# Aceinna/gnss-ins-sim

Hardware: NVIDIA H100
Metric: MC-runs x timesteps/sec free_integration @100Hz (higher is better)
Workload: dtype f64

## Files before the change

gnss_ins_sim_b200/csrc/b2ins_api.cu:

```cuda
#include <cmath>
#include <cstdarg>
#include <cstdio>
#include <cstdlib>
#include <cstring>
#include <limits>
#include <vector>

#include "../../include/b2ins.h"
#include "allan_kernel.cuh"
#include "internal.h"
#include "noise_kernel.cuh"
#include "pathgen_host.h"
#include "psd_kernel.cuh"
#include "gps_kernel.cuh"
#include "mag_kernel.cuh"
#include "ekf_kernel.cuh"
#include "stats_kernel.cuh"
#include "sensor_stats_kernel.cuh"

#ifdef B2INS_SINGLE_TU
#define B2_RF 0
#define B2_PLAIN_NAME launch_mc_plain_rf0
#define B2_SPEC_NAME launch_mc_spec_rf0
#include "mc_plain_launch.cuh"
// ... 860 lines not shown
    p.p0[3 + c] = cfg->gps_stdv[c] * cfg->gps_stdv[c];
    p.p0[6 + c] = cfg->ini_att_std[c] * cfg->ini_att_std[c];
    p.p0[9 + c] = cfg->gyro_err.b_drift[c] * cfg->gyro_err.b_drift[c] + cfg->gyro_err.b[c] * cfg->gyro_err.b[c];
    p.p0[12 + c] = cfg->accel_err.b_drift[c] * cfg->accel_err.b_drift[c] + cfg->accel_err.b[c] * cfg->accel_err.b[c];
    const bool wg = std::isinf(cfg->gyro_err.b_corr[c]), wa = std::isinf(cfg->accel_err.b_corr[c]);
    p.ag[c] = wg ? 0.0 : p.gyro.gm_a[c];
    p.qg[c] = wg ? p.gyro.wd[c] * p.gyro.wd[c] : p.gyro.gm_b[c] * p.gyro.gm_b[c];
    p.aa[c] = wa ? 0.0 : p.accel.gm_a[c];
    p.qa[c] = wa ? p.accel.wd[c] * p.accel.wd[c] : p.accel.gm_b[c] * p.accel.gm_b[c];
    p.arw2dt[c] = cfg->gyro_err.rw[c] * cfg->gyro_err.rw[c] * p.dt;
    p.vrw2dt[c] = cfg->accel_err.rw[c] * cfg->accel_err.rw[c] * p.dt;
  }
  for (int c = 0; c < 9; ++c) p.ini[c] = cfg->ini[c];
  ARG_CHECK(cfg->vel_rw >= 0.0 && cfg->att_rw >= 0.0, "vel_rw and att_rw must be >= 0");
  p.qv_extra = cfg->vel_rw * cfg->vel_rw * p.dt;
  p.qphi_extra = cfg->att_rw * cfg->att_rw * p.dt;
  p.stats_start = cfg->stats_start;
  p.end_err = end_err;
  p.end_bias = end_bias;
  p.consist = consist;
  p.out_att = dump_att;
  p.out_pos = dump_pos;
  p.out_vel = dump_vel;
  p.out_wb = dump_wb;
  p.out_ab = dump_ab;
  p.dump_runs = ndump ? cfg->dump_runs : 0;
  p.dump_stride = cfg->dump_stride > 1 ? cfg->dump_stride : 1;
  p.dump_rows = (cfg->n + p.dump_stride - 1) / p.dump_stride;
  const unsigned grid = static_cast<unsigned>((cfg->runs + kEkfRuns - 1) / kEkfRuns);
  ekf_kernel<<<grid, kEkfThreads, 0, static_cast<cudaStream_t>(stream)>>>(p);
  CU_CHECK(cudaGetLastError());
  return B2INS_OK;
}

int64_t b2ins_error_stats_workspace_bytes(int ncomp) {
  if (ncomp < 1) return 0;
  return static_cast<int64_t>(sizeof(double)) * (static_cast<int64_t>(kStatBlocks) * 2 + 4) * ncomp;
}

static int stage1_grid(int64_t runs, int ncomp, int threads) {
  const int64_t total = runs * ncomp;
  int64_t g = (total + threads - 1) / threads;
  if (g > kStatBlocks) g = kStatBlocks;
  if (g < 1) g = 1;
  return static_cast<int>(g);
}

int b2ins_error_partial_f64(int64_t runs, int ncomp, const double* err, double* partial,
                            void* workspace, void* stream) {
  ARG_CHECK(runs > 0 && ncomp >= 1 && ncomp <= kStatMaxComp, "bad runs/ncomp");
  ARG_CHECK(err && partial && workspace, "null buffer");
  cudaStream_t s = static_cast<cudaStream_t>(stream);
  const int threads = stat_threads(ncomp);
  const int grid = stage1_grid(runs, ncomp, threads);
  double* ws = static_cast<double*>(workspace);
  err_stage1_kernel<0><<<grid, threads, 2 * threads * sizeof(double), s>>>(runs, ncomp, err,
                                                                           nullptr, ws);
  err_stage2_kernel<0><<<1, 32, 0, s>>>(grid, ncomp, ws, partial);
  CU_CHECK(cudaGetLastError());
  return B2INS_OK;
}

int b2ins_error_partial2_f64(int64_t runs, int ncomp, const double* err, const double* mean,
                             double* partial2, void* workspace, void* stream) {
  ARG_CHECK(runs > 0 && ncomp >= 1 && ncomp <= kStatMaxComp, "bad runs/ncomp");
  ARG_CHECK(err && mean && partial2 && workspace, "null buffer");
  cudaStream_t s = static_cast<cudaStream_t>(stream);
  const int threads = stat_threads(ncomp);
  const int grid = stage1_grid(runs, ncomp, threads);
  double* ws = static_cast<double*>(workspace);
  err_stage1_kernel<1><<<grid, threads, 2 * threads * sizeof(double), s>>>(runs, ncomp, err, mean,
                                                                           ws);
  err_stage2_kernel<1><<<1, 32, 0, s>>>(grid, ncomp, ws, partial2);
  CU_CHECK(cudaGetLastError());
  return B2INS_OK;
}

int b2ins_error_stats_f64(int64_t runs, int ncomp, const double* err, double* stats,
                          void* workspace, void* stream) {
  ARG_CHECK(runs > 0 && ncomp >= 1 && ncomp <= kStatMaxComp, "bad runs/ncomp");
  ARG_CHECK(err && stats && workspace, "null buffer");
  cudaStream_t s = static_cast<cudaStream_t>(stream);
  if (runs * ncomp <= kStatSmallMax) {
    stats_small_kernel<<<1, kStatSmallThreads, 0, s>>>(runs, ncomp, err, stats);
    CU_CHECK(cudaGetLastError());
    return B2INS_OK;
  }
  double* ws = static_cast<double*>(workspace);
  double* partial = ws + static_cast<int64_t>(kStatBlocks) * 2 * ncomp;
  double* partial2 = partial + 2 * ncomp;
  int rc = b2ins_error_partial_f64(runs, ncomp, err, partial, workspace, stream);
  if (rc != B2INS_OK) return rc;
  stats_mean_kernel<<<1, 32, 0, s>>>(runs, ncomp, partial, stats);
  rc = b2ins_error_partial2_f64(runs, ncomp, err, stats + ncomp, partial2, workspace, stream);
  if (rc != B2INS_OK) return rc;
  stats_std_kernel<<<1, 32, 0, s>>>(runs, ncomp, partial2, stats);
  CU_CHECK(cudaGetLastError());
  return B2INS_OK;
}

int b2ins_error_stats_exchange_f64(int64_t runs, int ncomp, const double* err, int rank, int world,
                                   const uint64_t* windows, uint64_t seq, double* stats,
                                   int* timeout_flag, void* stream) {
  ARG_CHECK(runs >= 0 && ncomp >= 1 && 3 * ncomp + 2 <= kXchgSlot, "bad runs/ncomp");
  ARG_CHECK(runs * ncomp <= kStatSmallMax, "the fused exchange handles runs*ncomp <= 2^17 per rank");
  ARG_CHECK(world >= 1 && world <= kXchgMaxWorld && rank >= 0 && rank < world, "bad rank/world");
  ARG_CHECK(windows && stats && timeout_flag && seq >= 1, "null buffer / seq must start at 1");
  ARG_CHECK(runs == 0 || err, "null err");
  XchgParams p;
  std::memset(&p, 0, sizeof(p));
  p.runs = runs;
  p.ncomp = ncomp;
  p.rank = rank;
  p.world = world;
  p.seq = seq;
  p.err = err;
  for (int q = 0; q < world; ++q) p.peer[q] = reinterpret_cast<double*>(windows[q]);
  p.out = stats;
  p.timeout_flag = timeout_flag;
  stats_exchange_kernel<<<1, kStatSmallThreads, 0, static_cast<cudaStream_t>(stream)>>>(p);
  CU_CHECK(cudaGetLastError());
  return B2INS_OK;
}

int64_t b2ins_allan_workspace_bytes(int64_t n, int64_t nseries) {
  return allan_workspace_bytes(n, nseries);
}

int b2ins_allan_f64(double fs, int64_t n, int64_t nseries, const double* x, int64_t inner,
                    int64_t outer_stride, int64_t sample_stride, double* avar, double* tau,
                    void* workspace, void* stream) {
  ARG_CHECK(fs > 0.0 && n >= 0 && nseries >= 0, "bad fs/n/nseries");
  ARG_CHECK(inner >= 1 && sample_stride >= 1, "bad strides");
  int64_t mult[128];
  const int ntau = b2ins_allan_num_tau(n, fs, mult, 128);
  if (ntau == 0 || nseries == 0) return B2INS_OK;
  ARG_CHECK(ntau <= 128, "too many tau");
  ARG_CHECK(x && avar && tau && workspace, "null buffer");
  cudaStream_t s = static_cast<cudaStream_t>(stream);
  const int rc = allan_launch(fs, n, nseries, x, inner, outer_stride, sample_stride, mult, ntau,
                              avar, tau, workspace, sm_count(), s);
  if (rc != 0) return fail(B2INS_ERR_CUDA, "allan launch failed: %s", cudaGetErrorString(cudaGetLastError()));
  CU_CHECK(cudaGetLastError());
  return B2INS_OK;
}

int b2ins_allan_mc_f64(double fs, int64_t n, int64_t runs, const double* ref_gyro,
                       const double* ref_accel, const b2ins_sensor_err* gyro_err,
                       const b2ins_sensor_err* accel_err, uint64_t seed, int64_t run_offset,
                       double* avar, double* tau, void* workspace, void* stream) {
  ARG_CHECK(fs > 0.0 && n >= 0 && runs >= 0, "bad fs/n/runs");
  int64_t mult[128];
  const int ntau = b2ins_allan_num_tau(n, fs, mult, 128);
  if (ntau == 0 || runs == 0) return B2INS_OK;
  ARG_CHECK(ntau <= 128, "too many tau");
  ARG_CHECK(n > kAllanChunk, "the fused Allan path needs more than %d samples per series", kAllanChunk);
  ARG_CHECK(n < (int64_t(1) << 32), "n must be < 2^32");
  ARG_CHECK(ref_gyro && ref_accel && gyro_err && accel_err && avar && tau && workspace, "null buffer");
  AllanGenParams g;
  std::memset(&g, 0, sizeof(g));
  g.n = n;
  g.run_offset = run_offset;
  g.k0 = static_cast<uint32_t>(seed);
  g.k1 = static_cast<uint32_t>(seed >> 32);
  int rc = digest_triad(gyro_err, nullptr, fs, &g.gyro);
  if (rc != B2INS_OK) return rc;
  rc = digest_triad(accel_err, nullptr, fs, &g.accel);
  if (rc != B2INS_OK) return rc;
// ... 202 lines not shown
```

gnss_ins_sim_b200/csrc/common.cuh:

```cuda
#pragma once
#include <cstdint>
#include <cuda_runtime.h>

#include "fastmath64.cuh"

namespace b2ins {

constexpr double kRe = 6378137.0;
constexpr double kFlat = 1.0 / 298.257223563;
constexpr double kEcc = 0.0818191908426215;
constexpr double kESqr = kEcc * kEcc;
constexpr double kWie = 7292115e-11;
constexpr double kNormalGravity = 9.7803253359;
constexpr double kGravK = 0.00193185265241;
constexpr double kGravM = 0.00344978650684;
constexpr double kPi = 3.141592653589793238462643383279502884;
constexpr double kTwoPi = 2.0 * kPi;
constexpr double kHalfPi = 0.5 * kPi;

constexpr uint32_t kPhiloxM0 = 0xD2511F53u;
constexpr uint32_t kPhiloxM1 = 0xCD9E8D57u;
constexpr uint32_t kPhiloxW0 = 0x9E3779B9u;
constexpr uint32_t kPhiloxW1 = 0xBB67AE85u;

constexpr uint32_t kDrawAccel = 0;
constexpr uint32_t kDrawGyro = 3;
constexpr uint32_t kDrawVib = 6;
constexpr uint32_t kDrawPhase = 9;
constexpr uint32_t kDrawOdo = 12;
constexpr uint32_t kDrawMag = 13;
constexpr uint32_t kDrawPsd = 16;

struct PhiloxOut {
  uint32_t x0, x1, x2, x3;
};

__device__ __forceinline__ PhiloxOut philox4x32_10(uint32_t c0, uint32_t c1, uint32_t c2,
                                                   uint32_t c3, uint32_t k0, uint32_t k1) {
#pragma unroll
  for (int r = 0; r < 10; ++r) {
    const uint32_t hi0 = __umulhi(kPhiloxM0, c0), lo0 = kPhiloxM0 * c0;
    const uint32_t hi1 = __umulhi(kPhiloxM1, c2), lo1 = kPhiloxM1 * c2;
    const uint32_t n0 = hi1 ^ c1 ^ k0;
    const uint32_t n2 = hi0 ^ c3 ^ k1;
    c0 = n0;
    c1 = lo1;
    c2 = n2;
    c3 = lo0;
    k0 += kPhiloxW0;
    k1 += kPhiloxW1;
  }
  return PhiloxOut{c0, c1, c2, c3};
}

__device__ __forceinline__ double u01_from_bits(uint32_t lo, uint32_t hi) {
  const uint32_t mh = hi >> 12;
  const uint32_t ml = (hi << 20) | (lo >> 12);
  return __hiloint2double(0x3FF00000u | mh, ml) - 1.0;
}
__device__ __forceinline__ double one_plus_u01_from_bits(uint32_t lo, uint32_t hi) {
  const uint32_t mh = hi >> 12;
  const uint32_t ml = (hi << 20) | (lo >> 12);
  return __hiloint2double(0x3FF00000u | mh, ml);
}

struct Normal2 {
  double z0, z1;
};

__device__ __forceinline__ Normal2 normal_pair(uint32_t t, uint32_t draw, uint32_t run_lo,
                                               uint32_t run_hi, uint32_t k0, uint32_t k1) {
  const PhiloxOut x = philox4x32_10(t, draw, run_lo, run_hi, k0, k1);
  const double u1 = 2.0 - one_plus_u01_from_bits(x.x0, x.x1);
  const double r = sqrt_nr(-2.0 * log_unit(u1));
  double s, c;
  sincospi_2u(fma(one_plus_u01_from_bits(x.x2, x.x3), 2.0, -2.0), &s, &c);
  return Normal2{r * c, r * s};
}

__device__ __forceinline__ double uniform01(uint32_t t, uint32_t draw, uint32_t run_lo,
                                            uint32_t run_hi, uint32_t k0, uint32_t k1) {
  const PhiloxOut x = philox4x32_10(t, draw, run_lo, run_hi, k0, k1);
  return u01_from_bits(x.x0, x.x1);
}

__device__ __forceinline__ uint32_t smem_u32(const void* p) {
  return static_cast<uint32_t>(__cvta_generic_to_shared(p));
}
__device__ __forceinline__ void mbar_init(uint64_t* bar, uint32_t count) {
  asm volatile("mbarrier.init.shared::cta.b64 [%0], %1;" ::"r"(smem_u32(bar)), "r"(count));
}
__device__ __forceinline__ void mbar_fence_init() {
  asm volatile("fence.mbarrier_init.release.cluster;" ::: "memory");
  asm volatile("fence.proxy.async.shared::cta;" ::: "memory");
}
__device__ __forceinline__ void mbar_arrive(uint64_t* bar) {
  asm volatile("mbarrier.arrive.shared::cta.b64 _, [%0];" ::"r"(smem_u32(bar)) : "memory");
}
__device__ __forceinline__ void mbar_arrive_expect_tx(uint64_t* bar, uint32_t bytes) {
  asm volatile("mbarrier.arrive.expect_tx.shared::cta.b64 _, [%0], %1;" ::"r"(smem_u32(bar)),
               "r"(bytes)
               : "memory");
}
__device__ __forceinline__ void mbar_wait(uint64_t* bar, uint32_t parity) {
  asm volatile(
      "{\n"
      ".reg .pred p;\n"
      "WAIT_%=:\n"
      "mbarrier.try_wait.parity.shared::cta.b64 p, [%0], %1;\n"
      "@p bra DONE_%=;\n"
      "bra WAIT_%=;\n"
      "DONE_%=:\n"
      "}\n" ::"r"(smem_u32(bar)),
      "r"(parity)
      : "memory");
}
__device__ __forceinline__ void bulk_g2s(void* dst_smem, const void* src_gmem, uint32_t bytes,
                                         uint64_t* bar) {
  asm volatile(
      "cp.async.bulk.shared::cluster.global.mbarrier::complete_tx::bytes [%0], [%1], %2, [%3];" ::
          "r"(smem_u32(dst_smem)),
      "l"(src_gmem), "r"(bytes), "r"(smem_u32(bar))
      : "memory");
}
__device__ __forceinline__ void bulk_s2g(void* dst_gmem, const void* src_smem, uint32_t bytes) {
  asm volatile("cp.async.bulk.global.shared::cta.bulk_group [%0], [%1], %2;" ::"l"(dst_gmem),
               "r"(smem_u32(src_smem)), "r"(bytes)
               : "memory");
}
__device__ __forceinline__ void bulk_commit() {
  asm volatile("cp.async.bulk.commit_group;" ::: "memory");
}
__device__ __forceinline__ void bulk_wait_read0() {
  asm volatile("cp.async.bulk.wait_group.read 0;" ::: "memory");
}
__device__ __forceinline__ void bulk_wait0() {
  asm volatile("cp.async.bulk.wait_group 0;" ::: "memory");
}
__device__ __forceinline__ void fence_async_smem() {
  asm volatile("fence.proxy.async.shared::cta;" ::: "memory");
}

__host__ __device__ __forceinline__ int64_t min64(int64_t a, int64_t b) { return a < b ? a : b; }

template <int W>
__device__ __forceinline__ double shfl_grp(double v, int src) {
  return __shfl_sync(0xffffffffu, v, src, W);
}

}
```

gnss_ins_sim_b200/csrc/mc_av_kernel.cuh:

```cuda
#pragma once
#include <type_traits>

#include "mc_spec_kernel.cuh"

namespace b2ins {

constexpr int kAvRound = 8;
static_assert(kAvRound % kSpecBlock == 0, "A's rounds are whole speculative blocks");
template <int G>
struct AvShape {
  static constexpr int kHalves = (32 / G) / 4;
  static constexpr int kProd = 6 * kHalves;
  static constexpr int kWarps = (G == 4) ? 16 : 12;
  static constexpr int kSync = 32 * (2 + kProd);
};
__device__ constexpr int kAvRole8[12] = {-1, -2, 0, 1, -3, 2, 3, 4, -3, 5, -3, -3};
__device__ constexpr int kAvRole4[16] = {-1, -2, 0, 1, 2, 3, 4, 5, -3, 6, 7, 8, -3, 9, 10, 11};


template <int G>
struct AvSmem {
  alignas(128) double gyro[kStagesFast][kTile * 3];
  alignas(128) double accel[kStagesFast][kTile * 3];
  alignas(16) SampleSlot slot[3][kAvRound / G][32];
  alignas(16) double ring[2][kAvRound][32 / G][6];
  alignas(8) uint64_t full[kStagesFast];
  alignas(8) uint64_t empty[kStagesFast];
};

template <int G>
__global__ void __launch_bounds__(AvShape<G>::kWarps * 32, 1) mc_av_kernel(const __grid_constant__ McParams p) {
  static_assert(G == 4 || G == 8, "groups of 4 or 8 lanes");
  constexpr int kRunsPerCta = 32 / G;
  constexpr int kProd = AvShape<G>::kProd;
  constexpr int kAvSync = AvShape<G>::kSync;
  __shared__ AvSmem<G> sm;
  const int lane = threadIdx.x & 31;
  const int pwarp = threadIdx.x >> 5;
  const int role_w = (G == 4) ? kAvRole4[pwarp] : kAvRole8[pwarp];
  const bool is_a = role_w == -1, is_v = role_w == -2, is_p = role_w >= 0;
  const int pp = is_p ? role_w : 0;
  const int j = is_p ? (lane & 7) : lane % G;
  const int grp = is_p ? (pp / 6) * 4 + (lane >> 3) : lane / G;
  const McRun mr = mc_run(p, static_cast<int64_t>(blockIdx.x) * kRunsPerCta + grp);
  const int64_t num_tiles = (p.n + kTile - 1) / kTile;
  const int issuer = 2 * 32;
  auto stage_sync = [&]() { asm volatile("bar.sync 1, %0;" ::"n"(kAvSync) : "memory"); };

  if (threadIdx.x == 0) {
    for (int s = 0; s < kStagesFast; ++s) {
      mbar_init(&sm.full[s], 1);
      mbar_init(&sm.empty[s], kProd);
    }
    mbar_fence_init();
  }
#ifdef B2INS_PHASE_CLOCKS
  if (p.debug) {
    for (int q = threadIdx.x; q < static_cast<int>(sizeof(sm.slot) / 8); q += blockDim.x)
      reinterpret_cast<double*>(sm.slot)[q] = 0.0;
    for (int q = threadIdx.x; q < static_cast<int>(sizeof(sm.ring) / 8); q += blockDim.x)
      reinterpret_cast<double*>(sm.ring)[q] = 0.0;
  }
#endif
  __syncthreads();
  if (!is_a && !is_v && !is_p) return;
  const int64_t rounds = (p.n + kAvRound - 1) / kAvRound;

  if (is_p) {
    if (threadIdx.x == issuer)
      for (int s = 0; s < kStagesFast && s < num_tiles; ++s) issue_tile<false, false>(sm, p, s, s);
    const int c = pp % 6, ax = c % 3;
    const bool is_acc = c < 3;
    const TriadNoise& e = is_acc ? p.accel : p.gyro;
    const double eb = e.b[ax], ew = e.w[ax], ewd = e.wd[ax], ga = e.gm_a[ax], gb = e.gm_b[ax];
    double carry = 0.0;
    const double apj = ipow(ga, j), aG = ipow(ga, kAvRound);
    double phase[3] = {0.0, 0.0, 0.0};
    if (p.gyro.vib_type == 2) {
#pragma unroll
      for (int k = 0; k < 3; ++k)
        phase[k] = (uniform01(0xFFFFFFFFu, kDrawPhase + k, mr.lo, mr.hi, p.k0, p.k1) * 2.0) * kPi;
    }
    const bool any_vib = (p.accel.vib_type | p.gyro.vib_type) != 0;
    const double* ref0 = (is_acc ? sm.accel[0] : sm.gyro[0]) + j * 3 + ax;
    SampleSlot& slot0 = sm.slot[0][j / G][grp * G + (j % G)];
    double* out0 = (is_acc ? slot0.a : slot0.g) + ax;
    constexpr int kSlotSet = static_cast<int>(sizeof(sm.slot[0]) / sizeof(double));
    const int nrounds = static_cast<int>(rounds);
    const int ntiles = static_cast<int>(num_tiles);
    auto produce = [&](auto slow) {
      constexpr bool kSlow = decltype(slow)::value;
      int tile = 0, s = 0, base = 0, ref_off = 0, out_off = 0;
      uint32_t parity = 0, t0 = 0;
      int cnt = static_cast<int>(min64(kTile, p.n));
      for (int i = 0; i < nrounds; ++i) {
        if (base == 0) refill_and_wait<false, false>(sm, p, threadIdx.x == issuer, tile, ntiles, s, parity, 13);
        B2_CLK(cp0);
#ifdef B2INS_PHASE_CLOCKS
        if (!(p.debug & 1))
#endif
        {
          const int tj = base + j;
          const uint32_t t = t0 + static_cast<uint32_t>(tj);
          const bool live = tj < cnt;
          Normal2 z{0.0, 0.0};
          double m = 0.0;
          if (live) {
            z = normal_pair(t, c, mr.lo, mr.hi, p.k0, p.k1);
            m = (ref0[ref_off] + eb) + ew * z.z1;
            if (kSlow && any_vib)
              m += vib_term(e, ax, is_acc ? 0 : 1, t, mr.lo, mr.hi, p.k0, p.k1, mr.run, phase);
          }
          const double d = gm_block<kAvRound>(gb * z.z0, ga, apj, aG, j, carry);
          m += d + ewd * z.z0;
          int64_t row;
          if (kSlow && mr.warp_dumps && mr.dump && live && p.out_gyro && dump_row(p, t, &row))
            (is_acc ? p.out_accel : p.out_gyro)[mr.run * p.osr + row * p.ost + ax * p.osc] = m;
          out0[out_off] = m;
        }
        B2_CLK(cp1);
        B2_ACC(14, cp0, cp1);
        if (base + kAvRound >= cnt) {
          __syncwarp();
          if (lane == 0) mbar_arrive(&sm.empty[s]);
          ++tile;
          if (++s == kStagesFast) {
            s = 0;
            parity ^= 1u;
          }
          base = 0;
          t0 += kTile;
          ref_off = s * kTile * 3;
          cnt = static_cast<int>(min64(kTile, p.n - static_cast<int64_t>(t0)));
        } else {
          base += kAvRound;
          ref_off += kAvRound * 3;
        }
        out_off = (out_off == 2 * kSlotSet) ? 0 : out_off + kSlotSet;
// ... 138 lines not shown
```

gnss_ins_sim_b200/csrc/mc_kernel.cuh:

```cuda
#pragma once
#include "mech.cuh"

namespace b2ins {

constexpr int kPhaseClocks = 16;
#ifdef B2INS_PHASE_CLOCKS
__device__ unsigned long long g_phase_clocks[kPhaseClocks];
#define B2_CLK(var) const long long var = clock64()
#define B2_ACC(i, t0, t1) \
  if ((threadIdx.x & 31) == 0) atomicAdd(&g_phase_clocks[i], static_cast<unsigned long long>((t1) - (t0)))
#else
#define B2_CLK(var)
#define B2_ACC(i, t0, t1)
#endif

constexpr int kWarps = 4;
constexpr int kThreads = kWarps * 32;
constexpr int kTile = 128;
constexpr int kStagesFast = 3;
template <bool PROC>
struct Stages {
  static constexpr int value = PROC ? 2 : kStagesFast;
};

// ... 310 lines not shown
    const Vec3 xr = lla2ecef(r[3], r[4], r[5]);
    const Vec3 d{x.x - xr.x, x.y - xr.y, x.z - xr.z};
    if (pos_frame == 1) {
      double sl, cl, so, co;
      sincos_angle(r[3], &sl, &cl);
      sincos_angle(r[4], &so, &co);
      e[3] = -sl * co * d.x - sl * so * d.y + cl * d.z;
      e[4] = -so * d.x + co * d.y;
      e[5] = -cl * co * d.x - cl * so * d.y - sl * d.z;
    } else {
      e[3] = d.x;
      e[4] = d.y;
      e[5] = d.z;
    }
  } else {
    e[3] = st.pos.x - r[3];
    e[4] = st.pos.y - r[4];
    e[5] = st.pos.z - r[5];
  }
  e[6] = st.vel.x - r[6];
  e[7] = st.vel.y - r[7];
  e[8] = st.vel.z - r[8];
  if (pe_cnt == 0) {
#pragma unroll
    for (int c = 0; c < 9; ++c) pe_k[c] = e[c];
  }
#pragma unroll
  for (int c = 0; c < 9; ++c) {
    pe_max[c] = fmax(pe_max[c], fabs(e[c]));
    const double d = e[c] - pe_k[c];
    pe_sum[c] += d;
    pe_sq[c] += d * d;
  }
  ++pe_cnt;
}

__device__ __forceinline__ double ipow(double a, int e) {
  double r = 1.0, b = a;
#pragma unroll
  for (int bit = 0; bit < 6; ++bit) {
    if ((e >> bit) & 1) r *= b;
    b *= b;
  }
  return r;
}

#ifndef B2INS_G1_MINBLOCKS
#define B2INS_G1_MINBLOCKS 5
#endif
template <int G>
struct MinBlocks {
  static constexpr int value = (G == 1) ? B2INS_G1_MINBLOCKS : (G == 2 ? 3 : 2);
};

template <int G, int RF, bool FED, bool PROC>
__global__ void __launch_bounds__(kThreads, MinBlocks<G>::value)
mc_kernel(const __grid_constant__ McParams p) {
  __shared__ TileSmem<PROC> sm;
  constexpr int kRunsPerWarp = 32 / G;
  constexpr bool kSplit = (G >= 4);
  const int lane = threadIdx.x & 31;
  const int warp = threadIdx.x >> 5;
  const int j = lane % G;
  const int role = lane & 3;
  const McRun mr = mc_run(p, (static_cast<int64_t>(blockIdx.x) * kWarps + warp) * kRunsPerWarp + lane / G);
  const bool odo_mode = p.algo == 1;
  constexpr bool kStaged = !FED || PROC;
  constexpr int kStages = Stages<PROC>::value;

  const int64_t num_tiles = (p.n + kTile - 1) / kTile;
  if (kStaged) {
    if (threadIdx.x == 0) {
      for (int s = 0; s < kStages; ++s) {
        mbar_init(&sm.full[s], 1);
        mbar_init(&sm.empty[s], kWarps);
      }
      mbar_fence_init();
    }
    __syncthreads();
    if (threadIdx.x == 0) {
      for (int s = 0; s < kStages && s < num_tiles; ++s) issue_tile<FED, PROC>(sm, p, s, s);
    }
  }

  NavState st = mc_init<RF>(p, mr.run);
  double carry[6] = {0.0, 0.0, 0.0, 0.0, 0.0, 0.0};
  double apj[6], aG[6];
#pragma unroll
  for (int c = 0; c < 3; ++c) {
    const double aa = p.accel.gm_a[c], ag = p.gyro.gm_a[c];
    apj[c] = (G > 1) ? ipow(aa, j) : 1.0;
    apj[3 + c] = (G > 1) ? ipow(ag, j) : 1.0;
    aG[c] = (G > 1) ? ipow(aa, G) : aa;
    aG[3 + c] = (G > 1) ? ipow(ag, G) : ag;
  }
  double phase[3] = {0.0, 0.0, 0.0};
  if (!FED && p.gyro.vib_type == 2) {
#pragma unroll
    for (int c = 0; c < 3; ++c)
      phase[c] = (uniform01(0xFFFFFFFFu, kDrawPhase + c, mr.lo, mr.hi, p.k0, p.k1) * 2.0) * kPi;
  }
  if (mr.dump && j == 0 && p.out_att) put_state_row(p, mr.run, 0, st.yaw, st.pitch, st.roll, st.pos, st.vel);
  double pe_max[9], pe_sum[9], pe_sq[9], pe_k[9];
  int64_t pe_cnt = 0;
  if (PROC) {
#pragma unroll
    for (int c = 0; c < 9; ++c) pe_max[c] = pe_sum[c] = pe_sq[c] = pe_k[c] = 0.0;
  }

  for (int64_t tile = 0; tile < num_tiles; ++tile) {
    const int s = static_cast<int>(tile % kStages);
    const uint32_t parity = static_cast<uint32_t>((tile / kStages) & 1);
    const int64_t t0 = tile * kTile;
    const int cnt = static_cast<int>(min64(kTile, p.n - t0));
    if (kStaged)
      refill_and_wait<FED, PROC>(sm, p, threadIdx.x == 0, static_cast<int>(tile),
                                 static_cast<int>(num_tiles), s, parity, 0);

    for (int base = 0; base < cnt; base += G) {
      B2_CLK(ca0);
      double mg[3], ma[3];
      double mo = 0.0;
      const int tj = base + j;
      const int64_t t = t0 + tj;
      {
      if (FED) {
        if (tj < cnt) {
          const int64_t o = mr.run * p.sr + t * p.st;
#pragma unroll
          for (int c = 0; c < 3; ++c) {
            mg[c] = p.fed_gyro[o + c * p.sc];
            ma[c] = odo_mode ? 0.0 : p.fed_accel[o + c * p.sc];
          }
          if (odo_mode) mo = p.fed_odo[mr.run * p.so_r + t * p.so_t];
        } else {
#pragma unroll
          for (int c = 0; c < 3; ++c) mg[c] = ma[c] = 0.0;
        }
      } else {
        double zg[3], za[3];
        if (tj < cnt) {
          noisy_sample(p, &sm.accel[s][tj * 3], &sm.gyro[s][tj * 3], static_cast<uint32_t>(t), mr.lo,
                       mr.hi, mr.run, phase, ma, mg, za, zg);
        } else {
#pragma unroll
          for (int c = 0; c < 3; ++c) mg[c] = ma[c] = zg[c] = za[c] = 0.0;
        }
        B2_CLK(ca1);
        B2_ACC(1, ca0, ca1);
#pragma unroll
        for (int c = 0; c < 3; ++c) {
          const double da = gm_block<G>(p.accel.gm_b[c] * za[c], p.accel.gm_a[c], apj[c], aG[c], j,
                                        carry[c]);
          const double dg = gm_block<G>(p.gyro.gm_b[c] * zg[c], p.gyro.gm_a[c], apj[3 + c],
                                        aG[3 + c], j, carry[3 + c]);
          ma[c] += da + p.accel.wd[c] * za[c];
          mg[c] += dg + p.gyro.wd[c] * zg[c];
        }
        if (odo_mode) {
          const double zo = (tj < cnt) ? normal_pair(static_cast<uint32_t>(t), kDrawOdo, mr.lo, mr.hi,
                                                     p.k0, p.k1).z0 : 0.0;
          mo = (tj < cnt) ? p.odo_scale * p.ref_odo[t] + p.odo_stdv * zo : 0.0;
        }
      }
      int64_t row;
      if (mr.warp_dumps && mr.dump && tj < cnt && p.out_gyro && dump_row(p, t, &row)) {
// ... 93 lines not shown
```

gnss_ins_sim_b200/csrc/mc_spec_kernel.cuh:

```cuda
#pragma once
#include "mc_kernel.cuh"

namespace b2ins {

template <int G, int P, int WI>
struct SpecShape {
  static constexpr int kRound = (G >= 8) ? G : 8;
  static constexpr int kPasses = kRound / G;
  static constexpr bool kSpare = (P == 6 && WI == 1);
  static constexpr int kThreads = (WI * (1 + P) + (kSpare ? 1 : 0)) * 32;
  static constexpr int kChan = 6 / P;
  static constexpr bool kSpec = (G == 4 || G == 8);
  static_assert(6 % P == 0 && kTile % kRound == 0 && 32 % G == 0, "shape");
};

template <int G, int P, int WI>
struct SpecSmem {
  alignas(128) double gyro[kStagesFast][kTile * 3];
  alignas(128) double accel[kStagesFast][kTile * 3];
  alignas(16) SampleSlot slot[2][SpecShape<G, P, WI>::kPasses][WI][32];
  alignas(16) NavState saved[SpecShape<G, P, WI>::kSpec ? WI : 1][SpecShape<G, P, WI>::kSpec ? 32 : 1];
  alignas(8) uint64_t full[kStagesFast];
  alignas(8) uint64_t empty[kStagesFast];
};

template <int G, int RF, int P, int WI, bool SPLIT, int MINB>
__global__ void __launch_bounds__(SpecShape<G, P, WI>::kThreads, MINB)
mc_spec_kernel(const __grid_constant__ McParams p) {
  using Sh = SpecShape<G, P, WI>;
  static_assert(!SPLIT || G >= 4, "lane roles need groups of four");
  __shared__ SpecSmem<G, P, WI> sm;
  constexpr int kRunsPerWarp = 32 / G;
  constexpr int kChan = Sh::kChan;
  const int lane = threadIdx.x & 31;
  const int pwarp = threadIdx.x >> 5;
  const bool integrator = pwarp < WI;
  const int pidx = Sh::kSpare ? (pwarp < 4 ? pwarp - 1 : pwarp - 2) : pwarp - WI;
  const int gi = integrator ? pwarp : pidx / P;
  const int pp = integrator ? 0 : pidx % P;
  const int j = lane % G;
  const int role = lane & 3;
  const McRun mr = mc_run(p, (static_cast<int64_t>(blockIdx.x) * WI + gi) * kRunsPerWarp + lane / G);
  const int64_t num_tiles = (p.n + kTile - 1) / kTile;
  const int issuer = WI * 32;
  auto group_sync = [&]() { asm volatile("bar.sync %0, %1;" ::"r"(1 + gi), "n"(32 * (1 + P)) : "memory"); };

  if (threadIdx.x == 0) {
    for (int s = 0; s < kStagesFast; ++s) {
      mbar_init(&sm.full[s], 1);
      mbar_init(&sm.empty[s], WI * P);
    }
    mbar_fence_init();
  }
  __syncthreads();
  if (Sh::kSpare && pwarp == 4) return;

  if (!integrator) {
    if (threadIdx.x == issuer)
      for (int s = 0; s < kStagesFast && s < num_tiles; ++s) issue_tile<false, false>(sm, p, s, s);
    double carry[kChan], apj[kChan], aG[kChan];
#pragma unroll
    for (int q = 0; q < kChan; ++q) {
      const int c = pp * kChan + q;
      const double a = (c < 3) ? p.accel.gm_a[c % 3] : p.gyro.gm_a[c % 3];
      carry[q] = 0.0;
      apj[q] = (G > 1) ? ipow(a, j) : 1.0;
      aG[q] = (G > 1) ? ipow(a, G) : a;
    }
    double phase[3] = {0.0, 0.0, 0.0};
    if (p.gyro.vib_type == 2) {
#pragma unroll
      for (int c = 0; c < 3; ++c)
        phase[c] = (uniform01(0xFFFFFFFFu, kDrawPhase + c, mr.lo, mr.hi, p.k0, p.k1) * 2.0) * kPi;
    }
    const bool any_vib = (p.accel.vib_type | p.gyro.vib_type) != 0;
    int rnd = 0;
    for (int64_t tile = 0; tile < num_tiles; ++tile) {
      const int s = static_cast<int>(tile % kStagesFast);
      const uint32_t parity = static_cast<uint32_t>((tile / kStagesFast) & 1);
      const int64_t t0 = tile * kTile;
      const int cnt = static_cast<int>(min64(kTile, p.n - t0));
      refill_and_wait<false, false>(sm, p, threadIdx.x == issuer, static_cast<int>(tile),
                                    static_cast<int>(num_tiles), s, parity, 0);
      for (int base = 0; base < cnt; base += Sh::kRound, ++rnd) {
        const int buf = rnd & 1;
        B2_CLK(cp0);
#ifdef B2INS_PHASE_CLOCKS
        if (p.debug & 1) { group_sync(); continue; }
#endif
        constexpr int kIlp = (G >= 4 && Sh::kPasses >= 2) ? 2 : 1;
#pragma unroll 1
        for (int b0 = 0; b0 < Sh::kPasses; b0 += kIlp) {
          Normal2 z[kIlp][kChan];
#pragma unroll
          for (int bi = 0; bi < kIlp; ++bi)
#pragma unroll
            for (int q = 0; q < kChan; ++q) {
              z[bi][q] = Normal2{0.0, 0.0};
              if (kIlp > 1 || base + (b0 + bi) * G + j < cnt)
                z[bi][q] = normal_pair(static_cast<uint32_t>(t0 + base + (b0 + bi) * G + j), pp * kChan + q, mr.lo,
                                       mr.hi, p.k0, p.k1);
            }
#pragma unroll
          for (int bi = 0; bi < kIlp; ++bi) {
            const int b = b0 + bi;
            const int tj = base + b * G + j;
            const int64_t t = t0 + tj;
            const bool live = tj < cnt;
            SampleSlot& mine = sm.slot[buf][b][gi][lane];
#pragma unroll
            for (int q = 0; q < kChan; ++q) {
              const int c = pp * kChan + q;
              const int ax = c % 3;
              const bool is_acc = c < 3;
              const TriadNoise& e = is_acc ? p.accel : p.gyro;
              const double z0 = (kIlp > 1 && !live) ? 0.0 : z[bi][q].z0;
              double m = 0.0;
              if (live) {
                const double ref = is_acc ? sm.accel[s][tj * 3 + ax] : sm.gyro[s][tj * 3 + ax];
                m = (ref + e.b[ax]) + e.w[ax] * z[bi][q].z1;
                if (any_vib)
                  m += vib_term(e, ax, is_acc ? 0 : 1, static_cast<uint32_t>(t), mr.lo, mr.hi, p.k0, p.k1,
                                mr.run, phase);
              }
              const double d = gm_block<G>(e.gm_b[ax] * z0, e.gm_a[ax], apj[q], aG[q], j, carry[q]);
              m += d + e.wd[ax] * z0;
              int64_t row;
              if (mr.warp_dumps && mr.dump && live && p.out_gyro && dump_row(p, t, &row))
                (is_acc ? p.out_accel : p.out_gyro)[mr.run * p.osr + row * p.ost + ax * p.osc] = m;
              if (is_acc) mine.a[ax] = m; else mine.g[ax] = m;
            }
          }
        }
        B2_CLK(cp1);
        B2_ACC(7, cp0, cp1);
        group_sync();
// ... 81 lines not shown
```

gnss_ins_sim_b200/csrc/stats_kernel.cuh:

```cuda
#pragma once
#include "common.cuh"

namespace b2ins {

constexpr int kStatBlocks = 128;
constexpr int kStatMaxComp = 32;

__host__ __device__ inline int stat_threads(int ncomp) { return ncomp * (1024 / ncomp >= 32 ? 32 : 1024 / ncomp); }

template <int MODE>
__global__ void err_stage1_kernel(int64_t runs, int ncomp, const double* __restrict__ err,
                                  const double* __restrict__ mean, double* __restrict__ ws) {
  extern __shared__ double sh[];
  const int threads = blockDim.x;
  const int c = threadIdx.x % ncomp;
  const int64_t total = runs * ncomp;
  const int64_t stride = static_cast<int64_t>(gridDim.x) * threads;
  double acc = 0.0, mx = 0.0;
  const double mu = (MODE == 1) ? mean[c] : 0.0;
  for (int64_t i = static_cast<int64_t>(blockIdx.x) * threads + threadIdx.x; i < total; i += stride) {
    const double e = err[i];
    if (MODE == 0) {
      acc += e;
      mx = fmax(mx, fabs(e));
    } else {
      const double d = e - mu;
      acc += d * d;
    }
  }
  sh[threadIdx.x] = acc;
  sh[threads + threadIdx.x] = mx;
  __syncthreads();
  if (threadIdx.x < ncomp) {
    double s = 0.0, m = 0.0;
    for (int k = threadIdx.x; k < threads; k += ncomp) {
      s += sh[k];
      m = fmax(m, sh[threads + k]);
    }
    ws[(static_cast<int64_t>(blockIdx.x) * 2) * ncomp + c] = s;
    ws[(static_cast<int64_t>(blockIdx.x) * 2 + 1) * ncomp + c] = m;
  }
}

template <int MODE>
__global__ void err_stage2_kernel(int nblocks, int ncomp, const double* __restrict__ ws,
                                  double* __restrict__ out) {
  const int c = threadIdx.x;
  if (c >= ncomp) return;
  double s = 0.0, m = 0.0;
  for (int b = 0; b < nblocks; ++b) {
    s += ws[(static_cast<int64_t>(b) * 2) * ncomp + c];
    m = fmax(m, ws[(static_cast<int64_t>(b) * 2 + 1) * ncomp + c]);
  }
  out[c] = s;
  if (MODE == 0) out[ncomp + c] = m;
}

__global__ void stats_mean_kernel(int64_t runs, int ncomp, const double* __restrict__ partial,
                                  double* __restrict__ stats) {
  const int c = threadIdx.x;
  if (c >= ncomp) return;
  stats[c] = partial[ncomp + c];
  stats[ncomp + c] = partial[c] / static_cast<double>(runs);
}
__global__ void stats_std_kernel(int64_t runs, int ncomp, const double* __restrict__ partial2,
                                 double* __restrict__ stats) {
  const int c = threadIdx.x;
  if (c >= ncomp) return;
  stats[2 * ncomp + c] = sqrt(partial2[c] / static_cast<double>(runs));
}

constexpr int kStatSmallMax = 1 << 17;
constexpr int kStatSmallThreads = 1024;

__global__ void __launch_bounds__(kStatSmallThreads)
stats_small_kernel(int64_t runs, int ncomp, const double* __restrict__ err, double* __restrict__ stats) {
  __shared__ double sh[2 * kStatSmallThreads];
  __shared__ double mean_sh[kStatMaxComp];
  const int threads = (kStatSmallThreads / ncomp) * ncomp;
  const int c = threadIdx.x % ncomp;
  const int64_t total = runs * ncomp;
  const bool on = threadIdx.x < threads;
  double acc = 0.0, mx = 0.0;
  if (on)
    for (int64_t i = threadIdx.x; i < total; i += threads) {
      const double e = err[i];
      acc += e;
      mx = fmax(mx, fabs(e));
    }
  sh[threadIdx.x] = acc;
  sh[kStatSmallThreads + threadIdx.x] = mx;
  __syncthreads();
  if (threadIdx.x < ncomp) {
    double s = 0.0, m = 0.0;
    for (int k = threadIdx.x; k < threads; k += ncomp) {
      s += sh[k];
      m = fmax(m, sh[kStatSmallThreads + k]);
    }
    stats[c] = m;
    const double mean = s / static_cast<double>(runs);
    stats[ncomp + c] = mean;
    mean_sh[c] = mean;
  }
  __syncthreads();
  const double mu = mean_sh[c];
  acc = 0.0;
  if (on)
    for (int64_t i = threadIdx.x; i < total; i += threads) {
      const double d = err[i] - mu;
      acc += d * d;
    }
  sh[threadIdx.x] = acc;
  __syncthreads();
  if (threadIdx.x < ncomp) {
    double s = 0.0;
    for (int k = threadIdx.x; k < threads; k += ncomp) s += sh[k];
    stats[2 * ncomp + c] = sqrt(s / static_cast<double>(runs));
  }
}

constexpr int kXchgSlot = 32;
constexpr int kXchgMaxWorld = 16;

struct XchgParams {
  int64_t runs;
  int ncomp, rank, world;
  uint64_t seq;
  const double* err;
  double* peer[kXchgMaxWorld];
  double* out;
  int* timeout_flag;
};

__global__ void __launch_bounds__(kStatSmallThreads)
stats_exchange_kernel(const __grid_constant__ XchgParams p) {
  __shared__ double sh[2 * kStatSmallThreads];
  __shared__ double loc[3 * kStatMaxComp + 1];
  __shared__ int arrived[kXchgMaxWorld];
  const int nc = p.ncomp;
  const int threads = (kStatSmallThreads / nc) * nc;
  const int c = threadIdx.x % nc;
  const int64_t total = p.runs * nc;
  const bool on = threadIdx.x < threads;
  double acc = 0.0, mx = 0.0;
  if (on)
    for (int64_t i = threadIdx.x; i < total; i += threads) {
      const double e = p.err[i];
      acc += e;
      mx = fmax(mx, fabs(e));
    }
  sh[threadIdx.x] = acc;
  sh[kStatSmallThreads + threadIdx.x] = mx;
  __syncthreads();
  if (threadIdx.x < nc) {
    double s = 0.0, m = 0.0;
    for (int k = threadIdx.x; k < threads; k += nc) {
      s += sh[k];
      m = fmax(m, sh[kStatSmallThreads + k]);
    }
    loc[c] = m;
    loc[nc + c] = p.runs > 0 ? s / static_cast<double>(p.runs) : 0.0;
  }
  __syncthreads();
  const double mu = loc[nc + c];
  acc = 0.0;
  if (on)
    for (int64_t i = threadIdx.x; i < total; i += threads) {
      const double d = p.err[i] - mu;
      acc += d * d;
    }
  sh[threadIdx.x] = acc;
  __syncthreads();
  if (threadIdx.x < nc) {
    double s = 0.0;
    for (int k = threadIdx.x; k < threads; k += nc) s += sh[k];
    loc[2 * nc + c] = p.runs > 0 ? sqrt(s / static_cast<double>(p.runs)) : 0.0;
  }
  if (threadIdx.x == 0) loc[3 * nc] = static_cast<double>(p.runs);
  __syncthreads();
  const int par = static_cast<int>(p.seq & 1);
  const int64_t slot = (static_cast<int64_t>(par) * p.world + p.rank) * kXchgSlot;
  if (threadIdx.x <= 3 * nc) {
    const double v = loc[threadIdx.x];
    for (int q = 0; q < p.world; ++q) p.peer[q][slot + threadIdx.x] = v;
  }
  __threadfence_system();
  __syncthreads();
  if (threadIdx.x < p.world) {
    unsigned long long* f = reinterpret_cast<unsigned long long*>(p.peer[threadIdx.x] + slot + kXchgSlot - 1);
    asm volatile("st.release.sys.global.u64 [%0], %1;" ::"l"(f), "l"(p.seq) : "memory");
    const unsigned long long* mine = reinterpret_cast<const unsigned long long*>(
        p.peer[p.rank] + (static_cast<int64_t>(par) * p.world + threadIdx.x) * kXchgSlot + kXchgSlot - 1);
    unsigned long long seen = 0;
    const long long t0 = clock64();
    do {
      asm volatile("ld.acquire.sys.global.u64 %0, [%1];" : "=l"(seen) : "l"(mine) : "memory");
      if (clock64() - t0 > 40000000000LL) {
        *p.timeout_flag = 1;
        break;
      }
    } while (seen < p.seq);
// ... 30 lines not shown
```

Before: 6.865 billion.

## Overlap small stats kernel launch with MC kernel via PDL and register-cache errors

Launches the small stats kernel with programmatic stream serialization and has the MC kernels signal launch_dependents early, so the stats kernel's launch latency overlaps the tail of the integration kernel. The stats kernel now waits on griddepcontrol before reading, keeps up to nine error values per thread in registers so the variance pass needs no second global read, and splits the mean and max reductions across two warps using unrolled in-order folds. This removes launch gaps and repeated global loads. In exchange it adds early-resident stats blocks competing for SMs and uses 32-bit indexing for the total element count.

```diff
diff --git a/gnss_ins_sim_b200/csrc/b2ins_api.cu b/gnss_ins_sim_b200/csrc/b2ins_api.cu
--- a/gnss_ins_sim_b200/csrc/b2ins_api.cu
+++ b/gnss_ins_sim_b200/csrc/b2ins_api.cu
@@ -966,8 +966,16 @@
   ARG_CHECK(err && stats && workspace, "null buffer");
   cudaStream_t s = static_cast<cudaStream_t>(stream);
   if (runs * ncomp <= kStatSmallMax) {
-    stats_small_kernel<<<1, kStatSmallThreads, 0, s>>>(runs, ncomp, err, stats);
-    CU_CHECK(cudaGetLastError());
+    cudaLaunchConfig_t lc = {};
+    lc.gridDim = dim3(1);
+    lc.blockDim = dim3(kStatSmallThreads);
+    lc.stream = s;
+    cudaLaunchAttribute attr[1];
+    attr[0].id = cudaLaunchAttributeProgrammaticStreamSerialization;
+    attr[0].val.programmaticStreamSerializationAllowed = 1;
+    lc.attrs = attr;
+    lc.numAttrs = 1;
+    CU_CHECK(cudaLaunchKernelEx(&lc, stats_small_kernel, runs, ncomp, err, stats));
     return B2INS_OK;
   }
   double* ws = static_cast<double*>(workspace);
diff --git a/gnss_ins_sim_b200/csrc/common.cuh b/gnss_ins_sim_b200/csrc/common.cuh
--- a/gnss_ins_sim_b200/csrc/common.cuh
+++ b/gnss_ins_sim_b200/csrc/common.cuh
@@ -84,6 +84,9 @@
   return u01_from_bits(x.x0, x.x1);
 }
 
+__device__ __forceinline__ void launch_dependents() { asm volatile("griddepcontrol.launch_dependents;"); }
+__device__ __forceinline__ void grid_dependency_wait() { asm volatile("griddepcontrol.wait;" ::: "memory"); }
+
 __device__ __forceinline__ uint32_t smem_u32(const void* p) {
   return static_cast<uint32_t>(__cvta_generic_to_shared(p));
 }
diff --git a/gnss_ins_sim_b200/csrc/mc_av_kernel.cuh b/gnss_ins_sim_b200/csrc/mc_av_kernel.cuh
--- a/gnss_ins_sim_b200/csrc/mc_av_kernel.cuh
+++ b/gnss_ins_sim_b200/csrc/mc_av_kernel.cuh
@@ -54,6 +54,7 @@
     }
     mbar_fence_init();
   }
+  launch_dependents();
 #ifdef B2INS_PHASE_CLOCKS
   if (p.debug) {
     for (int q = threadIdx.x; q < static_cast<int>(sizeof(sm.slot) / 8); q += blockDim.x)
diff --git a/gnss_ins_sim_b200/csrc/mc_kernel.cuh b/gnss_ins_sim_b200/csrc/mc_kernel.cuh
--- a/gnss_ins_sim_b200/csrc/mc_kernel.cuh
+++ b/gnss_ins_sim_b200/csrc/mc_kernel.cuh
@@ -416,6 +416,7 @@
       for (int s = 0; s < kStages && s < num_tiles; ++s) issue_tile<FED, PROC>(sm, p, s, s);
     }
   }
+  launch_dependents();
 
   NavState st = mc_init<RF>(p, mr.run);
   double carry[6] = {0.0, 0.0, 0.0, 0.0, 0.0, 0.0};
diff --git a/gnss_ins_sim_b200/csrc/mc_spec_kernel.cuh b/gnss_ins_sim_b200/csrc/mc_spec_kernel.cuh
--- a/gnss_ins_sim_b200/csrc/mc_spec_kernel.cuh
+++ b/gnss_ins_sim_b200/csrc/mc_spec_kernel.cuh
@@ -52,6 +52,7 @@
     }
     mbar_fence_init();
   }
+  launch_dependents();
   __syncthreads();
   if (Sh::kSpare && pwarp == 4) return;
 
diff --git a/gnss_ins_sim_b200/csrc/stats_kernel.cuh b/gnss_ins_sim_b200/csrc/stats_kernel.cuh
--- a/gnss_ins_sim_b200/csrc/stats_kernel.cuh
+++ b/gnss_ins_sim_b200/csrc/stats_kernel.cuh
@@ -72,51 +72,99 @@
 
 constexpr int kStatSmallMax = 1 << 17;
 constexpr int kStatSmallThreads = 1024;
+constexpr int kStatKeep = 9;
+
+__device__ __forceinline__ double fold_in_order(const double* sh, int c, int step, int nb) {
+  double s = 0.0;
+  int b = 0;
+  if (nb >= 8) {
+    double x[8];
+#pragma unroll
+    for (int q = 0; q < 8; ++q) x[q] = sh[c + q * step];
+#pragma unroll 1
+    for (b = 8; b + 8 <= nb; b += 8) {
+      double y[8];
+#pragma unroll
+      for (int q = 0; q < 8; ++q) y[q] = sh[c + (b + q) * step];
+#pragma unroll
+      for (int q = 0; q < 8; ++q) s += x[q];
+#pragma unroll
+      for (int q = 0; q < 8; ++q) x[q] = y[q];
+    }
+#pragma unroll
+    for (int q = 0; q < 8; ++q) s += x[q];
+  }
+#pragma unroll 1
+  for (; b < nb; ++b) s += sh[c + b * step];
+  return s;
+}
+
+__device__ __forceinline__ double fold_max(const double* sh, int c, int step, int nb) {
+  double m[4] = {0.0, 0.0, 0.0, 0.0};
+  int b = 0;
+#pragma unroll 1
+  for (; b + 4 <= nb; b += 4) {
+#pragma unroll
+    for (int q = 0; q < 4; ++q) m[q] = fmax(m[q], sh[c + (b + q) * step]);
+  }
+#pragma unroll 1
+  for (; b < nb; ++b) m[0] = fmax(m[0], sh[c + b * step]);
+  return fmax(fmax(m[0], m[1]), fmax(m[2], m[3]));
+}
 
 __global__ void __launch_bounds__(kStatSmallThreads)
 stats_small_kernel(int64_t runs, int ncomp, const double* __restrict__ err, double* __restrict__ stats) {
   __shared__ double sh[2 * kStatSmallThreads];
   __shared__ double mean_sh[kStatMaxComp];
   const int threads = (kStatSmallThreads / ncomp) * ncomp;
-  const int c = threadIdx.x % ncomp;
-  const int64_t total = runs * ncomp;
-  const bool on = threadIdx.x < threads;
+  const int tid = threadIdx.x;
+  const int c = tid % ncomp;
+  const int total = static_cast<int>(runs) * ncomp;
+  const int mine = tid < threads ? (total - tid + threads - 1) / threads : 0;
+  const double* e0 = err + tid;
+  grid_dependency_wait();
+  double v[kStatKeep];
+#pragma unroll
+  for (int q = 0; q < kStatKeep; ++q) v[q] = q < mine ? e0[q * threads] : 0.0;
   double acc = 0.0, mx = 0.0;
-  if (on)
-    for (int64_t i = threadIdx.x; i < total; i += threads) {
-      const double e = err[i];
-      acc += e;
-      mx = fmax(mx, fabs(e));
-    }
-  sh[threadIdx.x] = acc;
-  sh[kStatSmallThreads + threadIdx.x] = mx;
-  __syncthreads();
-  if (threadIdx.x < ncomp) {
-    double s = 0.0, m = 0.0;
-    for (int k = threadIdx.x; k < threads; k += ncomp) {
-      s += sh[k];
-      m = fmax(m, sh[kStatSmallThreads + k]);
-    }
-    stats[c] = m;
-    const double mean = s / static_cast<double>(runs);
+#pragma unroll
+  for (int q = 0; q < kStatKeep; ++q)
+    if (q < mine) {
+      acc += v[q];
+      mx = fmax(mx, fabs(v[q]));
+    }
+  for (int q = kStatKeep; q < mine; ++q) {
+    const double e = e0[q * threads];
+    acc += e;
+    mx = fmax(mx, fabs(e));
+  }
+  sh[tid] = acc;
+  sh[kStatSmallThreads + tid] = mx;
+  __syncthreads();
+  if (tid < ncomp) {
+    const double mean = fold_in_order(sh, c, ncomp, threads / ncomp) / static_cast<double>(runs);
     stats[ncomp + c] = mean;
     mean_sh[c] = mean;
+  } else if (tid >= 32 && tid < 32 + ncomp) {
+    stats[tid - 32] = fold_max(sh + kStatSmallThreads, tid - 32, ncomp, threads / ncomp);
   }
   __syncthreads();
   const double mu = mean_sh[c];
   acc = 0.0;
-  if (on)
-    for (int64_t i = threadIdx.x; i < total; i += threads) {
-      const double d = err[i] - mu;
+#pragma unroll
+  for (int q = 0; q < kStatKeep; ++q)
+    if (q < mine) {
+      const double d = v[q] - mu;
       acc += d * d;
     }
-  sh[threadIdx.x] = acc;
-  __syncthreads();
-  if (threadIdx.x < ncomp) {
-    double s = 0.0;
-    for (int k = threadIdx.x; k < threads; k += ncomp) s += sh[k];
-    stats[2 * ncomp + c] = sqrt(s / static_cast<double>(runs));
-  }
+  for (int q = kStatKeep; q < mine; ++q) {
+    const double d = e0[q * threads] - mu;
+    acc += d * d;
+  }
+  sh[tid] = acc;
+  __syncthreads();
+  if (tid < ncomp)
+    stats[2 * ncomp + c] = sqrt(fold_in_order(sh, c, ncomp, threads / ncomp) / static_cast<double>(runs));
 }
 
 constexpr int kXchgSlot = 32;
```

Result: no change. 6.946 billion, median of 6 (+1.2%).
